# foxcroftjn/polars-strsim

Measured on AMD Instinct MI355X. Metric: M string-pairs/s, levenshtein, 100 M rows (+ achieved HBM GB/s in roofline), higher is better.
Workload: dtype u8/u32 bit-parallel, f64 epilogue

## Files before the change

polars-strsim_amd/csrc/strsim_lane_core.h:

```cpp
#pragma once
#include <stdint.h>
#include <type_traits>

#if defined(__HIPCC__)
#define STRSIM_HD __host__ __device__ __forceinline__
#else
#define STRSIM_HD inline
#endif

namespace strsim {

enum Measure : int { LEVENSHTEIN = 0, JARO = 1, JARO_WINKLER = 2, JACCARD = 3, SORENSEN_DICE = 4 };


#ifndef STRSIM_COLS_PER_TEST
#define STRSIM_COLS_PER_TEST 2
#endif
constexpr int COLS_PER_TEST = STRSIM_COLS_PER_TEST;

STRSIM_HD uint32_t lane_byte(const uint32_t (&w)[8], int j) { return (w[j >> 2] >> ((j & 3) * 8)) & 0xFFu; }

STRSIM_HD uint32_t low_ones(uint32_t k) { return k >= 32u ? 0xFFFFFFFFu : ((1u << k) - 1u); }

template <int G, int NG, typename F>
// ... 101 lines not shown
            const uint32_t t1 = perm_b32(w[2 + h], w[0 + h], 0x07030602u);
            const uint32_t t2 = perm_b32(w[6 + h], w[4 + h], 0x05010400u);
            const uint32_t t3 = perm_b32(w[6 + h], w[4 + h], 0x07030602u);
            r[4 * h + 0] = perm_b32(t2, t0, 0x05040100u);
            r[4 * h + 1] = perm_b32(t2, t0, 0x07060302u);
            r[4 * h + 2] = perm_b32(t3, t1, 0x05040100u);
            r[4 * h + 3] = perm_b32(t3, t1, 0x07060302u);
        }
    }
#pragma unroll
    for (int e = 0; e < 8; e += 2) {
        const uint32_t a = r[e], b = r[e + 1];
        r[e] = bitop3<0xCA>(0x55555555u, a, twice(b));
        r[e + 1] = bitop3<0xCA>(0x55555555u, a >> 1, b);
    }
#pragma unroll
    for (int q = 0; q < 4; ++q) {
        const int e = (q & 1) | ((q & 2) << 1);
        const uint32_t a = r[e], b = r[e + 2];
        r[e] = bitop3<0xCA>(0x33333333u, a, b << 2);
        r[e + 2] = bitop3<0xCA>(0x33333333u, a >> 2, b);
    }
#pragma unroll
    for (int e = 0; e < 4; ++e) {
        const uint32_t a = r[e], b = r[e + 4];
        if (e < NP) P[e < NP ? e : 0] = bitop3<0xCA>(0x0F0F0F0Fu, a, b << 4);
        if (e + 4 < NP) P[e + 4 < NP ? e + 4 : 0] = bitop3<0xCA>(0x0F0F0F0Fu, a >> 4, b);
    }
}

template <int NP>
STRSIM_HD uint32_t eq_mask(const uint32_t (&P)[NP], uint32_t valid, uint32_t w, int byte)
{
    uint32_t acc = valid;
#pragma unroll
    for (int k = 0; k < NP; ++k) acc = bitop3<0x90>(acc, P[k], bit_fill(w, 8 * byte + k));
    return acc;
}

STRSIM_HD int planes_needed(uint32_t vary) { return (vary & 0x40u) ? 7 : ((vary & 0x20u) ? 6 : 5); }

STRSIM_HD uint32_t window_vary(const uint32_t (&wa)[8], const uint32_t (&wb)[8], uint32_t &any)
{
    uint32_t o = bitop3<0xFE>(wa[0], wa[1], wa[2]), n = bitop3<0x80>(wa[0], wa[1], wa[2]);
    o = bitop3<0xFE>(o, wa[3], wa[4]); n = bitop3<0x80>(n, wa[3], wa[4]);
    o = bitop3<0xFE>(o, wa[5], wa[6]); n = bitop3<0x80>(n, wa[5], wa[6]);
    o = bitop3<0xFE>(o, wa[7], wb[0]); n = bitop3<0x80>(n, wa[7], wb[0]);
    o = bitop3<0xFE>(o, wb[1], wb[2]); n = bitop3<0x80>(n, wb[1], wb[2]);
    o = bitop3<0xFE>(o, wb[3], wb[4]); n = bitop3<0x80>(n, wb[3], wb[4]);
    o = bitop3<0xFE>(o, wb[5], wb[6]); n = bitop3<0x80>(n, wb[5], wb[6]);
    o |= wb[7]; n &= wb[7];
    uint32_t o8 = o | (o >> 16); o8 |= o8 >> 8;
    uint32_t n8 = n & (n >> 16); n8 &= n8 >> 8;
    any = o8 & 0xFFu;
    return (o8 ^ n8) & 0xFFu;
}

template <int NP>
STRSIM_HD uint32_t lev_myers32_snap(const uint32_t (&wt)[8], uint32_t lt, uint32_t tmin, uint32_t tmax, const uint32_t (&P)[NP],
                                    uint32_t lp)
{
    uint32_t Pv = 0xFFFFFFFFu, Mv = 0u;
#pragma unroll
    for (int g = 0; g < 32 / COLS_PER_TEST; ++g) {
        if ((uint32_t)(COLS_PER_TEST * g) >= tmax) break;
        auto column = [&](int j) {
            const uint32_t Eq = eq_mask<NP>(P, 0xFFFFFFFFu, wt[j >> 2], j & 3);
            const uint32_t D0 = bitop3<0xBE>((Eq & Pv) + Pv, Pv, Eq) | Mv;
            const uint32_t nHP = bitop3<0x0E>(Mv, D0, Pv);
            const uint32_t nX = twice(nHP);
            const uint32_t HN2 = twice(D0 & Pv);
            Pv = bitop3<0xF2>(HN2, D0, nX);
            Mv = bitop3<0x50>(D0, D0, nX);
        };
        if ((uint32_t)(COLS_PER_TEST * (g + 1)) >= tmin) {
#pragma unroll
            for (int jj = 0; jj < COLS_PER_TEST; ++jj)
                if ((uint32_t)(COLS_PER_TEST * g + jj) < lt) column(COLS_PER_TEST * g + jj);
        } else {
#pragma unroll
            for (int jj = 0; jj < COLS_PER_TEST; ++jj) column(COLS_PER_TEST * g + jj);
        }
    }
    const uint32_t rows = low_ones(lp);
    return lt + popc32(Pv & rows) - popc32(Mv & rows);
}

STRSIM_HD uint32_t common_prefix4(uint32_t a0, uint32_t la, uint32_t b0, uint32_t lb)
{
    const uint32_t x = a0 ^ b0;
    uint32_t p = 4u;
    if (x & 0x000000FFu) p = 0u;
    else if (x & 0x0000FF00u) p = 1u;
    else if (x & 0x00FF0000u) p = 2u;
    else if (x & 0xFF000000u) p = 3u;
    if (p > la) p = la;
    if (p > lb) p = lb;
    return p;
}

STRSIM_HD double epilogue_levenshtein(uint64_t dist, uint64_t la, uint64_t lb)
{
    const uint64_t den = la > lb ? la : lb;
    return 1.0 - ((double)dist / (double)den);
}

STRSIM_HD double epilogue_jaro(uint64_t m, uint64_t t, uint64_t la, uint64_t lb)
{
    if (m == 0) return 0.0;
    const double dm = (double)m;
    return (dm / (double)la + dm / (double)lb + (double)(m - t / 2) / dm) / 3.0;
}

STRSIM_HD double epilogue_jaro_winkler(double jaro, uint32_t prefix)
{
    if (jaro > 0.7) {
        const double pl = (double)prefix;
        return jaro + (pl * 0.1 * (1.0 - jaro));
    }
    return jaro;
}

STRSIM_HD double epilogue_jaccard(uint64_t isect, uint64_t la, uint64_t lb)
{
    return (double)isect / (double)(la + lb - isect);
}

STRSIM_HD double epilogue_sorensen_dice(uint64_t isect, uint64_t la, uint64_t lb)
{
    return 2.0 * (double)isect / (double)(la + lb);
}

template <int NP, bool DO_LEV, bool DO_JARO, bool DO_ISECT, bool KEEP_EQ = false>
STRSIM_HD void lane_cores32(const uint32_t (&wa)[8], uint32_t la, uint32_t tmin, uint32_t tmax, uint32_t lb,
                            const uint32_t (&P)[NP], uint32_t &dist, uint32_t &m_out, uint32_t &t_out, uint32_t &isect)
{
    const uint32_t lbmask = low_ones(lb);
    uint32_t Pv = 0xFFFFFFFFu, Mv = 0u;
    const uint32_t mx = la > lb ? la : lb;
    const uint32_t half = mx >> 1;
    const uint32_t bound = (half ? half : 1u) - 1u;
    uint32_t win = low_ones(bound + 1u);
    uint32_t fb = 0u, fa = 0u;
    const uint32_t valid = DO_JARO ? lbmask : 0xFFFFFFFFu;
    uint32_t used = 0u;
    uint32_t E[(DO_JARO && KEEP_EQ) ? 32 : 1];
#pragma unroll
    for (int g = 0; g < 32 / COLS_PER_TEST; ++g) {
        if ((uint32_t)(COLS_PER_TEST * g) >= tmax) break;
        auto column = [&](int i, bool live) {
            const uint32_t Eq = eq_mask<NP>(P, valid, wa[i >> 2], i & 3);
            if (DO_JARO && KEEP_EQ) E[(DO_JARO && KEEP_EQ) ? i : 0] = Eq;
            if (!live) return;
            if (DO_LEV) {
                const uint32_t D0 = bitop3<0xBE>((Eq & Pv) + Pv, Pv, Eq) | Mv;
                const uint32_t nHP = bitop3<0x0E>(Mv, D0, Pv);
                const uint32_t nX = twice(nHP);
                const uint32_t HN2 = twice(D0 & Pv);
                Pv = bitop3<0xF2>(HN2, D0, nX);
                Mv = bitop3<0x50>(D0, D0, nX);
            }
            if (DO_JARO) {
                const uint32_t cand = bitop3<0x40>(Eq, win, fb);
                fb = bitop3<0xF8>(fb, cand, 0u - cand);
                fa |= cand ? (1u << i) : 0u;
                win = win + win + ((uint32_t)i < bound ? 1u : 0u);
// ... 58 lines not shown
```

polars-strsim_amd/csrc/strsim_lane_stage.h:

```cpp
#pragma once

#ifndef STRSIM_STAGE_ROWS
#define STRSIM_STAGE_ROWS 512
#endif
#ifndef STRSIM_STAGE_CAP
#define STRSIM_STAGE_CAP 10240
#endif
#ifndef STRSIM_STAGE_CAP_LONG
#define STRSIM_STAGE_CAP_LONG 15104
#endif
#ifndef STRSIM_STAGE_CAP_LUT
#define STRSIM_STAGE_CAP_LUT 8960
#endif
#ifndef STRSIM_STAGE_WAVES_PER_EU
#define STRSIM_STAGE_WAVES_PER_EU 5
#endif
#ifndef STRSIM_STAGE_BUCKET_SHIFT
#define STRSIM_STAGE_BUCKET_SHIFT 1
#endif

#ifndef STRSIM_STAGE_LUT
#define STRSIM_STAGE_LUT 0x26
#endif
#ifndef STRSIM_JARO_KEEP_EQ_FILLS
#define STRSIM_JARO_KEEP_EQ_FILLS 1
#endif
#ifndef STRSIM_STAGE_LONG_TEXT_MAX
#define STRSIM_STAGE_LONG_TEXT_MAX 32
#endif
#ifndef STRSIM_STAGE_RANGE_MAX
#define STRSIM_STAGE_RANGE_MAX 64
#endif
#ifndef STRSIM_STAGE_RANGE_DIV
#define STRSIM_STAGE_RANGE_DIV 4
#endif
#ifndef STRSIM_STAGE_RANGE_MIN_BLOCKS
#define STRSIM_STAGE_RANGE_MIN_BLOCKS 2
#endif

#if defined(STRSIM_LAB) && defined(STRSIM_STAGE_STAMPS)
__device__ unsigned long long g_stage_stamps[16384][16];
#define STAGE_STAMP(cat) do { __builtin_amdgcn_sched_barrier(0); const unsigned long long t_ = __builtin_amdgcn_s_memtime(); \
                              __builtin_amdgcn_sched_barrier(0); st_acc[cat] += t_ - st_last; st_last = t_; } while (0)
#else
#define STAGE_STAMP(cat) do { } while (0)
#endif

#ifndef STRSIM_STAGE_THREADS
#define STRSIM_STAGE_THREADS 256
#endif
constexpr int STAGE_BLOCK = STRSIM_STAGE_THREADS;
constexpr int STAGE_WAVES = STAGE_BLOCK / 64;
constexpr int STAGE_ROWS = STRSIM_STAGE_ROWS;
constexpr int STAGE_RPT = STAGE_ROWS / STAGE_BLOCK;
constexpr int STAGE_NR = STAGE_ROWS / 64;
constexpr int STAGE_RPW = STAGE_NR / STAGE_WAVES;
template <int MEASURE> constexpr bool stage_uses_lut() { return ((STRSIM_STAGE_LUT >> MEASURE) & 1) != 0; }

template <bool TABLES, bool LONG = false> struct StageGeom {
    static_assert(!(TABLES && LONG), "the long-row geometry has no match-mask tables");
    static constexpr int CAP = LONG ? STRSIM_STAGE_CAP_LONG : (TABLES ? STRSIM_STAGE_CAP_LUT : STRSIM_STAGE_CAP);
    static constexpr int COL = CAP + 96;
    static constexpr int DMA_ITERS = (CAP + 48 + 16 * STAGE_BLOCK - 1) / (16 * STAGE_BLOCK);
    static_assert(CAP % 16 == 0 && 2 * COL + 64 + 16 <= 65536, "staging area: whole wave-instructions, 16-bit LDS offsets");
};
constexpr int STAGE_BSH = STRSIM_STAGE_BUCKET_SHIFT;
constexpr int STAGE_NBK = (32 >> STAGE_BSH) + 1;
static_assert(STAGE_RPT >= 1 && STAGE_RPT <= 4 && STAGE_RPW >= 1, "STAGE_ROWS is 256, 512 or 1024");
static_assert(STAGE_NBK <= 32, "the bucket scan runs on 32 lanes");

#define STRSIM_LDS_ADDR(p) ((uint32_t)(uintptr_t)((__attribute__((address_space(3))) void *)(p)))

__device__ __forceinline__ void lds_dma_b128(const void *gbase, uint32_t goff, uint32_t lds_dst)
{
    uint32_t keep;
    asm volatile("s_mov_b32 %0, m0\n\ts_mov_b32 m0, %3\n\ts_nop 0\n\tglobal_load_lds_dwordx4 %1, %2\n\ts_mov_b32 m0, %0"
                 : "=&s"(keep)
                 : "v"(goff), "s"(gbase), "s"(lds_dst)
                 : "memory");
}
__device__ __forceinline__ void lds_dma_b32(const void *gbase, uint32_t goff, uint32_t lds_dst)
{
    uint32_t keep;
    asm volatile("s_mov_b32 %0, m0\n\ts_mov_b32 m0, %3\n\ts_nop 0\n\tglobal_load_lds_dword %1, %2\n\ts_mov_b32 m0, %0"
                 : "=&s"(keep)
                 : "v"(goff), "s"(gbase), "s"(lds_dst)
                 : "memory");
}

__device__ __forceinline__ uint32_t load_invariant(const uint32_t *p)
{
    return *reinterpret_cast<const __attribute__((address_space(4))) uint32_t *>(reinterpret_cast<uintptr_t>(p));
}

constexpr uint32_t STAGE_DEAD = 1u << 31;

#if defined(STRSIM_LAB) && defined(STRSIM_STAGE_STRIP)
__device__ const uint16_t *g_strip_ptr;
__global__ __launch_bounds__(256) void k_strip_oracle(const uint32_t *__restrict__ offA, const uint8_t *__restrict__ valA, const uint32_t *__restrict__ offB,
                                                      const uint8_t *__restrict__ valB, uint64_t n, uint16_t *__restrict__ out)
{
    const uint64_t r = (uint64_t)blockIdx.x * 256u + threadIdx.x;
    if (r >= n) return;
    const uint32_t a0 = offA[r], la = offA[r + 1] - a0, b0 = offB[r], lb = offB[r + 1] - b0;
    const uint32_t m = la < lb ? la : lb, cap = (uint32_t)STRSIM_STAGE_STRIP;
    uint32_t p = 0, s = 0;
    while (p < m && p < cap && valA[a0 + p] == valB[b0 + p]) ++p;
    while (s < m - p && s < cap && valA[a0 + la - 1u - s] == valB[b0 + lb - 1u - s]) ++s;
    if (p + s > 63u) s = 63u - p;
    out[r] = (uint16_t)(p | (s << 8));
}
#define STRSIM_STRIP_ON 1
#else
#define STRSIM_STRIP_ON 0
#endif

__device__ __forceinline__ void stage_window(const uint8_t *base, uint32_t at, uint32_t (&w)[8], uint32_t lds_bytes = 0u, uint32_t who = 0u)
{
    typedef uint32_t u32x4_a4 __attribute__((ext_vector_type(4), aligned(4)));
    (void)lds_bytes; (void)who;
    if (who == 1u) STRSIM_CHECK_RANGE(K_STAGE, 40, ~0ull, (at & ~3u) + 36u, 0, lds_bytes);
    if (who == 2u) STRSIM_CHECK_RANGE(K_LIT, 40, ~0ull, (at & ~3u) + 36u, 0, lds_bytes);
    const uint8_t *q = base + (at & ~3u);
    const u32x4_a4 lo = *reinterpret_cast<const u32x4_a4 *>(q);
    const u32x4_a4 hi = *reinterpret_cast<const u32x4_a4 *>(q + 16);
    const uint32_t top = *reinterpret_cast<const uint32_t *>(q + 32);
    const uint32_t sh = at & 3u;
    w[0] = __builtin_amdgcn_alignbyte(lo.y, lo.x, sh); w[1] = __builtin_amdgcn_alignbyte(lo.z, lo.y, sh);
    w[2] = __builtin_amdgcn_alignbyte(lo.w, lo.z, sh); w[3] = __builtin_amdgcn_alignbyte(hi.x, lo.w, sh);
    w[4] = __builtin_amdgcn_alignbyte(hi.y, hi.x, sh); w[5] = __builtin_amdgcn_alignbyte(hi.z, hi.y, sh);
    w[6] = __builtin_amdgcn_alignbyte(hi.w, hi.z, sh); w[7] = __builtin_amdgcn_alignbyte(top, hi.w, sh);
}

__device__ __forceinline__ uint32_t scan32_inclusive(uint32_t x)
{
    x += (uint32_t)__builtin_amdgcn_update_dpp(0, (int)x, 0x111, 0xF, 0xF, true);
    x += (uint32_t)__builtin_amdgcn_update_dpp(0, (int)x, 0x112, 0xF, 0xF, true);
    x += (uint32_t)__builtin_amdgcn_update_dpp(0, (int)x, 0x114, 0xF, 0xF, true);
    x += (uint32_t)__builtin_amdgcn_update_dpp(0, (int)x, 0x118, 0xF, 0xF, true);
    x += (uint32_t)__builtin_amdgcn_update_dpp(0, (int)x, 0x142, 0xA, 0xF, true);
    return x;
}

template <int NP, bool USE_LUT>
__device__ __forceinline__ uint32_t stage_lev_code(const EqLut &lut, const uint32_t (&wa)[8], uint32_t la, const uint32_t (&wb)[8],
                                                   uint32_t lb, uint32_t tmin, uint32_t tmax, uint32_t stripped = 0u)
{
    uint32_t P[NP];
    build_planes<NP>(wb, P);
    EqLut t = lut;
    if (USE_LUT) lut_build<NP>(t, P, 0xFFFFFFFFu);
    const bool live = la != 0u && lb != 0u;
    const uint32_t la1 = live ? la : 1u, lb1 = live ? lb : 1u;
    const uint32_t dist = USE_LUT ? lev_myers32_lut<NP>(t, wa, la1, tmin, tmax, P, lb1) : lev_myers32_snap<NP>(wa, la1, tmin, tmax, P, lb1);
    uint32_t code = dist * (uint32_t)QTAB_N + (la1 > lb1 ? la1 : lb1);
    if (!live) code = (la == 0u && lb == 0u) ? 1u : (uint32_t)QTAB_N + 1u;
#if STRSIM_STRIP_ON
    const uint32_t longer = la > lb ? la : lb;
    code = (live ? dist : longer) * (uint32_t)QTAB_N + (longer + stripped);
#endif
    return code;
}

template <int NP, bool USE_LUT>
__device__ __forceinline__ unsigned long long stage_all_ints(const EqLut &lut, const uint32_t (&wa)[8], uint32_t la,
                                                             const uint32_t (&wb)[8], uint32_t lb, uint32_t tmin, uint32_t tmax)
{
    uint32_t P[NP];
    build_planes<NP>(wb, P);
    const bool live = la != 0u && lb != 0u;
    const uint32_t la1 = live ? la : 1u, lb1 = live ? lb : 1u;
    uint32_t dist, m, t, isect;
    if (USE_LUT) {
        EqLut tb = lut;
        lut_build<NP>(tb, P, 0xFFFFFFFFu);
        lane_cores32_lut<NP, true, true, true>(tb, wa, la1, tmin, tmax, lb1, P, dist, m, t, isect);
    } else {
        lane_cores32<NP, true, true, true>(wa, la1, tmin, tmax, lb1, P, dist, m, t, isect);
    }
    const uint32_t pre = common_prefix4(wa[0], la1, wb[0], lb1);
    const uint32_t lo = dist | (m << 6) | (t << 12) | (isect << 18) | (pre << 24) | (la << 27);
    return (unsigned long long)lo | ((unsigned long long)(la >> 5) << 32) | ((unsigned long long)lb << 33);
}

__device__ __forceinline__ void stage_all_epilogues(unsigned long long pk, double qa, double qb, double qc, double qd, double (&r)[5])
{
    const uint32_t lo = (uint32_t)pk, hi = (uint32_t)(pk >> 32);
    const uint32_t m = (lo >> 6) & 63u, isect = (lo >> 18) & 63u, pre = (lo >> 24) & 7u;
    const uint32_t la = ((lo >> 27) & 31u) | ((hi & 1u) << 5), lb = (hi >> 1) & 63u;
    if (la == 0u || lb == 0u) {
        const double v = (la == 0u && lb == 0u) ? 1.0 : 0.0;
#pragma unroll
        for (int q = 0; q < 5; ++q) r[q] = v;
        return;
    }
    r[LEVENSHTEIN] = 1.0 - qd;
    const double j = m == 0u ? 0.0 : div3_exact(qa + qb + qc);
    r[JARO] = j;
    r[JARO_WINKLER] = epilogue_jaro_winkler(j, pre);
    r[JACCARD] = epilogue_jaccard(isect, la, lb);
    r[SORENSEN_DICE] = epilogue_sorensen_dice(isect, la, lb);
}

template <int MEASURE, int NP, bool USE_LUT>
__device__ __forceinline__ uint32_t stage_ints(const EqLut &lut, const uint32_t (&wa)[8], uint32_t la, const uint32_t (&wb)[8],
                                               uint32_t lb, uint32_t tmin, uint32_t tmax)
{
    uint32_t P[NP];
    build_planes<NP>(wb, P);
    const bool live = la != 0u && lb != 0u;
    const uint32_t la1 = live ? la : 1u, lb1 = live ? lb : 1u;
    uint32_t dist, m, t, isect;
    EqLut tb = lut;
    if (USE_LUT) lut_build<NP>(tb, P, 0xFFFFFFFFu);
    if (MEASURE == JARO || MEASURE == JARO_WINKLER) {
        if (USE_LUT) lane_cores32_lut<NP, false, true, false>(tb, wa, la1, tmin, tmax, lb1, P, dist, m, t, isect);
        else lane_cores32<NP, false, true, false, STRSIM_JARO_KEEP_EQ_FILLS != 0>(wa, la1, tmin, tmax, lb1, P, dist, m, t, isect);
        const uint32_t pre = MEASURE == JARO_WINKLER ? common_prefix4(wa[0], la1, wb[0], lb1) : 0u;
        return m | (t << 6) | (la << 12) | (lb << 18) | (pre << 24);
    }
    if (USE_LUT) lane_cores32_lut<NP, false, false, true>(tb, wa, la1, tmin, tmax, lb1, P, dist, m, t, isect);
    else lane_cores32<NP, false, false, true>(wa, la1, tmin, tmax, lb1, P, dist, m, t, isect);
    return isect | (la << 6) | (lb << 12);
}

template <int MEASURE>
__device__ __forceinline__ double stage_epilogue(uint32_t pk, double qa, double qb, double qc)
{
    if (MEASURE == JARO || MEASURE == JARO_WINKLER) {
        const uint32_t m = pk & 63u, la = (pk >> 12) & 63u, lb = (pk >> 18) & 63u, pre = (pk >> 24) & 7u;
        if (la == 0u || lb == 0u) return (la == 0u && lb == 0u) ? 1.0 : 0.0;
        const double j = m == 0u ? 0.0 : div3_exact(qa + qb + qc);
        return MEASURE == JARO_WINKLER ? epilogue_jaro_winkler(j, pre) : j;
    }
    const uint32_t isect = pk & 63u, la = (pk >> 6) & 63u, lb = (pk >> 12) & 63u;
    if (la == 0u || lb == 0u) return (la == 0u && lb == 0u) ? 1.0 : 0.0;
    return MEASURE == JACCARD ? epilogue_jaccard(isect, la, lb) : epilogue_sorensen_dice(isect, la, lb);
}

template <int MEASURE, bool LUT>
__device__ __forceinline__ void stage_compute(const EqLut &lut, const uint32_t (&wt)[8], const uint32_t (&wp)[8], uint32_t meta,
                                              uint32_t last, uint16_t *s_code, uint32_t *s_word, double *s_val)
{
    bool fast = (meta & STAGE_DEAD) == 0u;
#if STRSIM_STRIP_ON
    const uint32_t lt = meta & 0x3Fu, lp = (meta >> 8) & 0x3Fu, idx = (meta >> 16) & 0x1FFu, stripped = (meta >> 25) & 0x3Fu;
#else
    const uint32_t lt = meta & 0x3Fu, lp = (meta >> 8) & 0x3Fu, idx = (meta >> 16) & 0x7FFu, stripped = 0u;
#endif
    uint32_t any;
    const uint32_t vary = window_vary(wt, wp, any);
    if (any & 0x80u) fast = false;
    if (__ballot(fast) == 0ull) return;
    const uint32_t la = fast ? lt : 0u, lb = fast ? lp : 0u;
    static_assert((1 << STAGE_BSH) % COLS_PER_TEST == 0, "a bucket's upper bound is a whole number of column groups");
    const uint32_t ltl = (uint32_t)__builtin_amdgcn_readlane((int)lt, (int)last);
    const uint32_t tmax = (((ltl ? ltl : 1u) - 1u) | ((1u << STAGE_BSH) - 1u)) + 1u;
    const bool wide = __ballot(fast && (vary & 0x60u)) != 0ull;
    const uint32_t lt0 = uniform(lt);
    const uint32_t tmin = (((lt0 ? lt0 : 1u) - 1u) & ~((1u << STAGE_BSH) - 1u)) + 1u;
    if (MEASURE == LEVENSHTEIN) {
        uint32_t code;
        if (wide) code = stage_lev_code<7, LUT>(lut, wt, la, wp, lb, tmin, tmax, stripped);
        else code = stage_lev_code<5, LUT>(lut, wt, la, wp, lb, tmin, tmax, stripped);
        if (fast) STRSIM_CHECK_INDEX(K_STAGE, 42, ~0ull, idx, STAGE_ROWS);
        if (fast) s_code[idx] = (uint16_t)code;
    } else if (MEASURE == ALL_MEASURES) {
        unsigned long long pk;
        if (wide) pk = stage_all_ints<7, LUT>(lut, wt, la, wp, lb, tmin, tmax);
        else pk = stage_all_ints<5, LUT>(lut, wt, la, wp, lb, tmin, tmax);
        if (fast) STRSIM_CHECK_INDEX(K_STAGE, 43, ~0ull, idx, STAGE_ROWS);
        if (fast) reinterpret_cast<unsigned long long *>(s_val)[idx] = pk;
    } else {
        uint32_t pk;
        if (wide) pk = stage_ints<MEASURE, 7, LUT>(lut, wt, la, wp, lb, tmin, tmax);
        else pk = stage_ints<MEASURE, 5, LUT>(lut, wt, la, wp, lb, tmin, tmax);
        if (fast) STRSIM_CHECK_INDEX(K_STAGE, 44, ~0ull, idx, STAGE_ROWS);
        if (fast) s_word[idx] = pk;
    }
}

template <int MEASURE, bool LUT, bool LONG = false>
__device__ __forceinline__ void
lane_stage_body(const uint32_t *__restrict__ offA, const uint8_t *__restrict__ valA, uint64_t rowsA,
             const uint32_t *__restrict__ offB, const uint8_t *__restrict__ valB, uint64_t rowsB, OutPtrs outs,
             uint64_t n, unsigned long long *__restrict__ slowmask, DevStatus *__restrict__ status,
             const double *__restrict__ qtab, uint32_t *__restrict__ sched, DevStatus *__restrict__ publish, uint32_t ticket)
{
    constexpr bool LEV = MEASURE == LEVENSHTEIN;
    constexpr bool ALL = MEASURE == ALL_MEASURES;
    constexpr int B = STAGE_ROWS, RPT = STAGE_RPT, NBK = STAGE_NBK;
    constexpr int STAGE_CAP = StageGeom<LUT, LONG>::CAP, STAGE_COL = StageGeom<LUT, LONG>::COL;
    constexpr int STAGE_DMA_ITERS = StageGeom<LUT, LONG>::DMA_ITERS;
    constexpr uint32_t COLB = STAGE_COL, LIT = 2u * STAGE_COL;
    static_assert(!LUT || (B <= 128 * STAGE_WAVES && LUT_WAVE_BYTES == 3072), "descriptor slices: 128 rows behind each wave's tables");
    __shared__ __attribute__((aligned(4096))) uint8_t s_lut[LUT ? 4096 * STAGE_WAVES : 16];
    __shared__ uint2 s_desc_own[LUT ? 1 : B];
    __shared__ __attribute__((aligned(4096))) uint8_t s_bytes[2 * STAGE_COL + 64 + 16];
    auto desc_at = [&](uint32_t p) -> uint2 * {
        if (LUT) return reinterpret_cast<uint2 *>(s_lut + ((p >> 7) << 12) + LUT_WAVE_BYTES + ((p & 127u) << 3));
        return s_desc_own + p;
    };
    __shared__ __attribute__((aligned(16))) uint32_t s_off[2][B + 4];
    __shared__ uint32_t s_cnt[32];
    __shared__ uint32_t s_left;
    __shared__ uint32_t s_sched[2];
    __shared__ uint16_t s_code[LEV ? B : 1];
    __shared__ uint32_t s_word[(!LEV && !ALL) ? B : 1];
    __shared__ double s_val[ALL ? B : 1];

    const uint32_t tid = threadIdx.x, lane = lane_id(), wv = tid >> 6;
    if (blockIdx.x == 0u && tid < (uint32_t)(sizeof(DevStatus) / sizeof(uint32_t))) reinterpret_cast<uint32_t *>(status)[tid] = 0u;
    if (tid < 32u) s_cnt[tid] = 0u;
    if (tid == 0u) s_left = 0u;
#pragma unroll
    for (int q = 0; q < RPT; ++q) {
        const uint32_t i = (uint32_t)q * STAGE_BLOCK + tid;
        if (LEV) s_code[i] = 0xFFFFu;
        else if (ALL) reinterpret_cast<unsigned long long *>(&s_val[i])[0] = ~0ull;
        else s_word[i] = 0xFFFFFFFFu;
    }

    const uint32_t totalA = load_invariant(offA + rowsA), totalB = load_invariant(offB + rowsB);
#if STRSIM_BOUNDS_ON
    const uint32_t firstA = load_invariant(offA), firstB = load_invariant(offB);
#endif
    const bool bcastA = rowsA == 1, bcastB = rowsB == 1;
    const uint32_t litA0 = bcastA ? load_invariant(offA) : 0u, litB0 = bcastB ? load_invariant(offB) : 0u;
    const uint32_t litAlen = bcastA ? totalA - litA0 : 0u, litBlen = bcastB ? totalB - litB0 : 0u;
    if (wv == 0u) {
        auto literal_window = [&](const uint8_t *val, uint32_t at, uint32_t total, uint32_t len, uint32_t *dst) {
            uint32_t w[8];
            load_window32(val, at, total, w);
            const uint32_t rep = (w[0] & 0xFFu) * 0x01010101u;
#pragma unroll
            for (int q = 0; q < 8; ++q) {
                const uint32_t v = len > 4u * q ? (len - 4u * q < 4u ? len - 4u * q : 4u) : 0u;
                const uint32_t keep = v >= 4u ? 0xFFFFFFFFu : ((1u << (8u * v)) - 1u);
                dst[q] = (w[q] & keep) | (rep & ~keep);
            }
        };
        if (bcastA) literal_window(valA, litA0, totalA, litAlen, reinterpret_cast<uint32_t *>(s_bytes + LIT));
        if (bcastB) literal_window(valB, litB0, totalB, litBlen, reinterpret_cast<uint32_t *>(s_bytes + LIT + 32u));
    }
    const uint64_t nchunks = (n + 63u) >> 6;
    const uint32_t nchunks32 = (uint32_t)nchunks;
    auto grab = [&](uint32_t seen, uint32_t &lo, uint32_t &sz) {
        const uint32_t left = nchunks32 > seen ? nchunks32 - seen : 0u;
        uint32_t want = (uint32_t)STRSIM_STAGE_RANGE_MAX;
        if (left < (uint32_t)(STRSIM_STAGE_RANGE_MAX * STRSIM_STAGE_RANGE_DIV) * gridDim.x) want = left / ((uint32_t)STRSIM_STAGE_RANGE_DIV * gridDim.x);
        sz = want < (uint32_t)(STRSIM_STAGE_RANGE_MIN_BLOCKS * (B / 64)) ? (uint32_t)(STRSIM_STAGE_RANGE_MIN_BLOCKS * (B / 64)) : want;
        lo = __hip_atomic_fetch_add(&sched[0], sz, __ATOMIC_RELAXED, __HIP_MEMORY_SCOPE_AGENT);
    };
    uint32_t grab_lo = 0u, grab_sz = 0u;
    if (tid == 0u) {
        grab(0u, grab_lo, grab_sz);
        s_sched[0] = grab_lo;
        s_sched[1] = grab_sz;
    }
    lds_barrier();
    uint64_t row_end;
    uint64_t row0;
    {
        const uint64_t lo = uniform(s_sched[0]), hi = lo + uniform(s_sched[1]);
        row0 = lo * 64u < n ? lo * 64u : n;
        row_end = hi * 64u < n ? hi * 64u : n;
    }
    lds_barrier();
    if (tid == 0u) grab(grab_lo, grab_lo, grab_sz);
    bool grab_pending = true;

    EqLut lut;
    lut.lane4 = lane * 4u;
    lut.krep = ((STRSIM_LDS_ADDR(&s_lut[0]) >> 8) + 16u * wv) * 0x01010101u;
    const uint32_t ldsOffA = STRSIM_LDS_ADDR(&s_off[0][0]), ldsOffB = STRSIM_LDS_ADDR(&s_off[1][0]);
    const uint32_t ldsBytes = STRSIM_LDS_ADDR(&s_bytes[0]);
    const uint32_t wvu = uniform(wv);
    const uint32_t tid4 = tid * 4u, tid16 = tid * 16u;
    auto dma_offsets = [&](uint64_t row) {
        const uint32_t cnt = (uint32_t)(row_end - row < (uint64_t)B ? row_end - row : (uint64_t)B);
        const uint32_t *const pa = offA + row, *const pb = offB + row;
#pragma unroll
        for (int it = 0; it < RPT; ++it) {
            if (tid + (uint32_t)it * STAGE_BLOCK <= cnt) {
                if (!bcastA) STRSIM_CHECK_INDEX(K_STAGE, 1, row, row + (uint64_t)it * STAGE_BLOCK + tid, rowsA + 1u);
                if (!bcastB) STRSIM_CHECK_INDEX(K_STAGE, 2, row, row + (uint64_t)it * STAGE_BLOCK + tid, rowsB + 1u);
                STRSIM_CHECK_INDEX(K_STAGE, 3, row, (uint32_t)it * STAGE_BLOCK + tid, B + 4);
                if (!bcastA) lds_dma_b32(pa + it * STAGE_BLOCK, tid4, ldsOffA + 4u * ((uint32_t)it * STAGE_BLOCK + wvu * 64u));
                if (!bcastB) lds_dma_b32(pb + it * STAGE_BLOCK, tid4, ldsOffB + 4u * ((uint32_t)it * STAGE_BLOCK + wvu * 64u));
            }
        }
        if (tid == 0u && cnt == (uint32_t)B) {
            if (!bcastA) STRSIM_CHECK_INDEX(K_STAGE, 4, row, row + (uint64_t)B, rowsA + 1u);
            if (!bcastB) STRSIM_CHECK_INDEX(K_STAGE, 5, row, row + (uint64_t)B, rowsB + 1u);
            if (!bcastA) lds_dma_b32(pa + B, tid4, ldsOffA + 4u * (uint32_t)B);
            if (!bcastB) lds_dma_b32(pb + B, tid4, ldsOffB + 4u * (uint32_t)B);
// ... 91 lines not shown
        }
    };

#if defined(STRSIM_LAB) && defined(STRSIM_STAGE_STAMPS)
    unsigned long long st_acc[10] = {0, 0, 0, 0, 0, 0, 0, 0, 0, 0};
    const unsigned long long st_t0 = __builtin_amdgcn_s_memtime(), st_r0 = __builtin_amdgcn_s_memrealtime();
    unsigned long long st_last = st_t0;
#endif
    while (row0 < row_end) {
        if (grab_pending) {
            if (tid == 0u) {
                s_sched[0] = grab_lo;
                s_sched[1] = grab_sz;
            }
            grab_pending = false;
        }
        if (prev_rows) store_block(prev_row0, prev_rows);
        STAGE_STAMP(1);
        const uint32_t avail = (uint32_t)(row_end - row0 < (uint64_t)B ? row_end - row0 : (uint64_t)B);
        const uint32_t baseA = bcastA ? litA0 : uniform(s_off[0][0]), baseB = bcastB ? litB0 : uniform(s_off[1][0]);
        const uint32_t misA = (uint32_t)(reinterpret_cast<uintptr_t>(valA + baseA) & 15u);
        const uint32_t misB = (uint32_t)(reinterpret_cast<uintptr_t>(valB + baseB) & 15u);
        uint32_t rows;
        {
            const uint32_t e = (lane + 1u) * 64u < avail ? (lane + 1u) * 64u : avail;
            const bool exists = lane * 64u < avail && lane < (uint32_t)(B / 64);
            const uint32_t endA = bcastA ? baseA : s_off[0][exists ? e : 0u], endB = bcastB ? baseB : s_off[1][exists ? e : 0u];
            const bool fits = exists && endA - baseA + misA <= (uint32_t)STAGE_CAP && endB - baseB + misB <= (uint32_t)STAGE_CAP;
            const unsigned long long okm = __ballot(fits);
            uint32_t k = (uint32_t)__builtin_ctzll(~okm);
            if (k == 0u) k = 1u;
            rows = uniform(k * 64u < avail ? k * 64u : avail);
        }
        const uint32_t endA = bcastA ? baseA : uniform(s_off[0][rows]), endB = bcastB ? baseB : uniform(s_off[1][rows]);
        const uint32_t spanA = endA - baseA + misA, spanB = endB - baseB + misB;
        const uint32_t stagedA = bcastA ? 0u : (((spanA < (uint32_t)STAGE_CAP ? spanA : (uint32_t)STAGE_CAP) + 15u) & ~15u);
        const uint32_t stagedB = bcastB ? 0u : (((spanB < (uint32_t)STAGE_CAP ? spanB : (uint32_t)STAGE_CAP) + 15u) & ~15u);
        const uint32_t leftA = totalA - baseA + misA, leftB = totalB - baseB + misB;
        const uint32_t chunksA = bcastA ? 0u : ((stagedA + 32u < leftA ? stagedA + 32u : leftA) + 15u) >> 4;
        const uint32_t chunksB = bcastB ? 0u : ((stagedB + 32u < leftB ? stagedB + 32u : leftB) + 15u) >> 4;
        if (tid < 2u) STRSIM_CHECK_RANGE(K_STAGE, 20, row0, (chunksA << 4) + tid * 16u + 16u, 0, COLB);
        else if (tid < 4u) STRSIM_CHECK_RANGE(K_STAGE, 21, row0, COLB + (chunksB << 4) + (tid - 2u) * 16u + 16u, 0, sizeof(s_bytes));
        if (tid < 2u) *reinterpret_cast<uint4 *>(s_bytes + (chunksA << 4) + tid * 16u) = make_uint4(0u, 0u, 0u, 0u);
        else if (tid < 4u) *reinterpret_cast<uint4 *>(s_bytes + COLB + (chunksB << 4) + (tid - 2u) * 16u) = make_uint4(0u, 0u, 0u, 0u);
        {
            const uint8_t *__restrict__ const gA = valA + baseA - misA, *__restrict__ const gB = valB + baseB - misB;
#pragma unroll
            for (int it = 0; it < STAGE_DMA_ITERS; ++it) {
                if (tid + (uint32_t)it * STAGE_BLOCK < chunksA) {
                    STRSIM_CHECK_COLUMN(K_STAGE, 22, row0, gA + 16 * it * STAGE_BLOCK + tid16, 16, valA, firstA, totalA);
                    STRSIM_CHECK_RANGE(K_STAGE, 23, row0, 16u * ((uint32_t)it * STAGE_BLOCK + tid) + 16u, 0, COLB);
                    lds_dma_b128(gA + 16 * it * STAGE_BLOCK, tid16, ldsBytes + 16u * ((uint32_t)it * STAGE_BLOCK + wvu * 64u));
                }
                if (tid + (uint32_t)it * STAGE_BLOCK < chunksB) {
                    STRSIM_CHECK_COLUMN(K_STAGE, 24, row0, gB + 16 * it * STAGE_BLOCK + tid16, 16, valB, firstB, totalB);
                    STRSIM_CHECK_RANGE(K_STAGE, 25, row0, COLB + 16u * ((uint32_t)it * STAGE_BLOCK + tid) + 16u, 0, sizeof(s_bytes));
                    lds_dma_b128(gB + 16 * it * STAGE_BLOCK, tid16, ldsBytes + COLB + 16u * ((uint32_t)it * STAGE_BLOCK + wvu * 64u));
                }
            }
        }
        STAGE_STAMP(0);
        uint32_t skey[RPT], srank[RPT], sd0[RPT], sd1[RPT];
        {
#pragma unroll
            for (int q = 0; q < RPT; ++q) {
                const uint32_t i = (uint32_t)RPT * tid + (uint32_t)q;
                STRSIM_CHECK_INDEX(K_STAGE, 30, row0, i + 1u, B + 4);
                const bool have = i < rows;
                const uint32_t a0 = bcastA ? 0u : s_off[0][i] - baseA, b0 = bcastB ? 0u : s_off[1][i] - baseB;
                const uint32_t la8 = bcastA ? litAlen : s_off[0][i + 1u] - s_off[0][i];
                const uint32_t lb8 = bcastB ? litBlen : s_off[1][i + 1u] - s_off[1][i];
                const bool stA = bcastA || misA + a0 + la8 <= stagedA, stB = bcastB || misB + b0 + lb8 <= stagedB;
                bool mine = have && la8 <= 32u && lb8 <= 32u && stA && stB;
                if (LONG && STRSIM_STAGE_LONG_TEXT_MAX < 32 && !bcastA && !bcastB) mine = mine && (la8 < lb8 ? la8 : lb8) <= (uint32_t)STRSIM_STAGE_LONG_TEXT_MAX;
                const uint32_t wa = bcastA ? LIT : misA + a0, wb = bcastB ? LIT + 32u : COLB + misB + b0;
                const bool swap = !bcastA && !bcastB && la8 > lb8;
#if STRSIM_STRIP_ON
                uint32_t sp = 0u, ss = 0u;
                if (LEV && !bcastA && !bcastB && have) {
                    const uint32_t ps = g_strip_ptr[row0 + i];
                    sp = ps & 0xFFu; ss = ps >> 8;
                }
                const uint32_t lt = (swap ? lb8 : la8) - sp - ss, lp = (swap ? la8 : lb8) - sp - ss;
                const uint32_t key = mine ? (((lt ? lt : 1u) - 1u) >> STAGE_BSH) : (uint32_t)(NBK - 1);
                skey[q] = key;
                srank[q] = atomicAdd(&s_cnt[key], 1u);
                sd0[q] = mine ? (swap ? ((wb + sp) | ((wa + sp) << 16)) : ((wa + sp) | ((wb + sp) << 16))) : 0u;
                sd1[q] = mine ? (lt | (lp << 8) | (i << 16) | ((sp + ss) << 25)) : STAGE_DEAD;
#else
                const uint32_t lt = swap ? lb8 : la8, lp = swap ? la8 : lb8;
                const uint32_t key = mine ? (((lt ? lt : 1u) - 1u) >> STAGE_BSH) : (uint32_t)(NBK - 1);
                skey[q] = key;
                srank[q] = atomicAdd(&s_cnt[key], 1u);
                sd0[q] = mine ? (swap ? (wb | (wa << 16)) : (wa | (wb << 16))) : 0u;
                sd1[q] = mine ? (lt | (lp << 8) | (i << 16)) : STAGE_DEAD;
#endif
            }
        }
        STAGE_STAMP(2);
        lds_barrier();
        STAGE_STAMP(3);
        uint32_t nmine;
        {
            const uint32_t c = s_cnt[lane & 31u];
            const uint32_t exc = scan32_inclusive(c) - c;
#pragma unroll
            for (int q = 0; q < RPT; ++q) {
                const uint32_t base = __shfl(exc, skey[q], 32);
                const uint32_t p = base + srank[q];
                STRSIM_CHECK_INDEX(K_STAGE, 31, row0, p, B);
                *desc_at(p) = make_uint2(sd0[q], sd1[q]);
            }
            nmine = uniform(__shfl(exc, NBK - 1, 32));
        }
        STAGE_STAMP(4);
        asm volatile("s_waitcnt vmcnt(0)" ::: "memory");
        if (!bcastA && leftA < (chunksA << 4) && tid == ((chunksA - 1u) & (uint32_t)(STAGE_BLOCK - 1)))
            for (uint32_t b = leftA; b < (chunksA << 4); ++b) { STRSIM_CHECK_INDEX(K_STAGE, 32, row0, b, COLB); s_bytes[b] = 0; }
        if (!bcastB && leftB < (chunksB << 4) && tid == ((chunksB - 1u) & (uint32_t)(STAGE_BLOCK - 1)))
            for (uint32_t b = leftB; b < (chunksB << 4); ++b) { STRSIM_CHECK_INDEX(K_STAGE, 33, row0, COLB + b, sizeof(s_bytes)); s_bytes[COLB + b] = 0; }
        lds_barrier();
        STAGE_STAMP(5);
        if (tid < 32u) s_cnt[tid] = 0u;
        uint64_t next_row0 = row0 + rows;
        if (next_row0 >= row_end) {
            const uint64_t lo = uniform(s_sched[0]), hi = lo + uniform(s_sched[1]);
            next_row0 = lo * 64u < n ? lo * 64u : n;
            row_end = hi * 64u < n ? hi * 64u : n;
            if (tid == 0u) grab((uint32_t)lo, grab_lo, grab_sz);
            grab_pending = true;
        }
        if (next_row0 < row_end) dma_offsets(next_row0);
        STAGE_STAMP(6);
        __builtin_amdgcn_s_setprio(0);
        {
            const uint32_t nrounds = (nmine + 63u) >> 6;
#pragma unroll 1
            for (int k = 0; k < STAGE_RPW; ++k) {
                const uint32_t t = (uint32_t)(k >> 1) * (2u * STAGE_WAVES) + ((k & 1) ? (uint32_t)(2 * STAGE_WAVES - 1) - wv : wv);
                if (t >= nrounds) continue;
                const uint32_t hi = nmine - 64u * t;
                const uint32_t first = hi >= 64u ? hi - 64u : 0u;
                const uint32_t in_round = hi - first;
                __builtin_amdgcn_s_setprio(1);
                STRSIM_CHECK_INDEX(K_STAGE, 41, row0, first + lane, B);
                const uint2 d = *desc_at(first + lane);
                uint32_t wt[8], wp[8];
                stage_window(s_bytes, d.x & 0xFFFFu, wt, (uint32_t)sizeof(s_bytes), STRSIM_BOUNDS_ON ? 1u : 0u);
                stage_window(s_bytes, d.x >> 16, wp, (uint32_t)sizeof(s_bytes), STRSIM_BOUNDS_ON ? 1u : 0u);
    #if defined(STRSIM_LAB) && defined(STRSIM_STAGE_STAMPS)
                asm volatile("s_waitcnt lgkmcnt(0)" ::: "memory");
    #endif
                STAGE_STAMP(7);
                __builtin_amdgcn_s_setprio(0);
                stage_compute<MEASURE, LUT>(lut, wt, wp, lane < in_round ? d.y : STAGE_DEAD, in_round - 1u, s_code, s_word, s_val);
                STAGE_STAMP(8);
            }
        }
        __builtin_amdgcn_s_setprio(1);
        asm volatile("s_waitcnt vmcnt(0)" ::: "memory");
        lds_barrier();
        STAGE_STAMP(9);
        prev_row0 = row0;
        prev_rows = rows;
        row0 = next_row0;
    }
    if (prev_rows) store_block(prev_row0, prev_rows);
    if (publish) lds_barrier();
    if (tid == 0u) {
        if (publish && s_left) __hip_atomic_fetch_add(&sched[2], s_left, __ATOMIC_RELAXED, __HIP_MEMORY_SCOPE_AGENT);
        const uint32_t done = __hip_atomic_fetch_add(&sched[1], 1u, __ATOMIC_ACQ_REL, __HIP_MEMORY_SCOPE_AGENT);
        if (done == gridDim.x - 1u) {
            if (publish) {
                const uint32_t total = __hip_atomic_load(&sched[2], __ATOMIC_RELAXED, __HIP_MEMORY_SCOPE_AGENT);
                __hip_atomic_store(&publish->lane_left, total, __ATOMIC_RELEASE, __HIP_MEMORY_SCOPE_SYSTEM);
                if (ticket) __hip_atomic_store(&publish->ticket, ticket, __ATOMIC_RELEASE, __HIP_MEMORY_SCOPE_SYSTEM);
            }
            __hip_atomic_store(&sched[0], 0u, __ATOMIC_RELAXED, __HIP_MEMORY_SCOPE_AGENT);
            __hip_atomic_store(&sched[1], 0u, __ATOMIC_RELAXED, __HIP_MEMORY_SCOPE_AGENT);
            __hip_atomic_store(&sched[2], 0u, __ATOMIC_RELAXED, __HIP_MEMORY_SCOPE_AGENT);
        }
    }
#if defined(STRSIM_LAB) && defined(STRSIM_STAGE_STAMPS)
    if (lane == 0u) {
        const uint32_t w = (blockIdx.x * STAGE_WAVES + wv) & 16383u;
        for (int q = 0; q < 10; ++q) g_stage_stamps[w][q] = st_acc[q];
        g_stage_stamps[w][10] = __builtin_amdgcn_s_memtime() - st_t0;
        const unsigned long long st_r1 = __builtin_amdgcn_s_memrealtime();
        g_stage_stamps[w][11] = st_r1 - st_r0;
        g_stage_stamps[w][12] = st_r0;
        g_stage_stamps[w][13] = st_r1;
        g_stage_stamps[w][14] = (unsigned long long)__builtin_amdgcn_s_getreg((4 << 0) | (0 << 6) | (31 << 11));
        g_stage_stamps[w][15] = (unsigned long long)__builtin_amdgcn_s_getreg((20 << 0) | (0 << 6) | (31 << 11));
    }
#endif
}

#ifndef STRSIM_STAGE_PLAIN_WAVES
#define STRSIM_STAGE_PLAIN_WAVES 5
#endif
#ifndef STRSIM_STAGE_ALL_WAVES_PER_EU
#define STRSIM_STAGE_ALL_WAVES_PER_EU 3
#endif
template <int MEASURE, bool TABLES, bool LONG = false> constexpr int stage_waves_per_eu()
{
    constexpr int lim = MEASURE == ALL_MEASURES ? STRSIM_STAGE_ALL_WAVES_PER_EU : ((TABLES || LONG) ? 4 : STRSIM_STAGE_PLAIN_WAVES);
    return STRSIM_STAGE_WAVES_PER_EU < lim ? STRSIM_STAGE_WAVES_PER_EU : lim;
}

template <int MEASURE, bool TABLES, bool LONG = false>
__global__ __launch_bounds__(STAGE_BLOCK) __attribute__((amdgpu_waves_per_eu(stage_waves_per_eu<MEASURE, TABLES, LONG>()))) void
k_lane_stage(const uint32_t *__restrict__ offA, const uint8_t *__restrict__ valA, uint64_t rowsA,
             const uint32_t *__restrict__ offB, const uint8_t *__restrict__ valB, uint64_t rowsB, OutPtrs outs, uint64_t n,
             unsigned long long *__restrict__ slowmask, DevStatus *__restrict__ status, const double *__restrict__ qtab,
             uint32_t *__restrict__ sched, DevStatus *__restrict__ publish, uint32_t ticket)
{
    lane_stage_body<MEASURE, TABLES, LONG>(offA, valA, rowsA, offB, valB, rowsB, outs, n, slowmask, status, qtab, sched, publish, ticket);
}

__global__ __launch_bounds__(STAGE_BLOCK) __attribute__((amdgpu_waves_per_eu(stage_waves_per_eu<ALL_MEASURES, stage_uses_lut<ALL_MEASURES>()>()))) void
k_lane_stage_all(const uint32_t *__restrict__ offA, const uint8_t *__restrict__ valA, uint64_t rowsA,
                 const uint32_t *__restrict__ offB, const uint8_t *__restrict__ valB, uint64_t rowsB, OutPtrs outs, uint64_t n,
                 unsigned long long *__restrict__ slowmask, DevStatus *__restrict__ status, const double *__restrict__ qtab,
                 uint32_t *__restrict__ sched, DevStatus *__restrict__ publish, uint32_t ticket)
{
    lane_stage_body<ALL_MEASURES, stage_uses_lut<ALL_MEASURES>()>(offA, valA, rowsA, offB, valB, rowsB, outs, n, slowmask, status, qtab, sched, publish, ticket);
}
```

Baseline: 70150.

## Sort Levenshtein rows by exact text length and mask columns per-lane suffix

For the Levenshtein non-LUT path, rows are now bucketed by exact text length (bucket shift 0, 33 buckets with a 64-lane scan) instead of 2-column buckets. The Myers loop becomes a fully unrolled column walk where, past the round's minimum length, each column's active lanes are computed from the bucket boundaries via readlane and an inverse ballot. Lanes whose text is already exhausted stop updating, so per-lane tail checks are replaced by wave-uniform masks. This is meant to tighten the tmin/tmax column range per wave. The cost is a wider count scan, an extra readlane per pair of columns, and loss of the COLS_PER_TEST grouping.

```diff
diff --git a/polars-strsim_amd/csrc/strsim_lane_core.h b/polars-strsim_amd/csrc/strsim_lane_core.h
--- a/polars-strsim_amd/csrc/strsim_lane_core.h
+++ b/polars-strsim_amd/csrc/strsim_lane_core.h
@@ -207,6 +207,40 @@
             for (int jj = 0; jj < COLS_PER_TEST; ++jj) column(COLS_PER_TEST * g + jj);
         }
     }
+    const uint32_t rows = low_ones(lp);
+    return lt + popc32(Pv & rows) - popc32(Mv & rows);
+}
+
+struct TailPerPair {
+    STRSIM_HD bool live(int j, uint32_t lt, uint32_t) { return (uint32_t)j < lt; }
+};
+
+STRSIM_HD unsigned long long suffix_live_mask(uint32_t pair, int j, uint32_t first)
+{
+    const int below = (int)((j & 1) ? pair >> 16 : pair & 0xFFFFu) - (int)first;
+    const int c = below > 0 ? below : 0;
+    return below >= 64 ? 0ull : ~0ull << (uint32_t)c;
+}
+
+template <int NP, typename TAIL>
+STRSIM_HD uint32_t lev_myers32_ordered(const uint32_t (&wt)[8], uint32_t lt, uint32_t tmin, uint32_t tmax, const uint32_t (&P)[NP],
+                                       uint32_t lp, TAIL tail)
+{
+    uint32_t Pv = 0xFFFFFFFFu, Mv = 0u;
+    unrolled_until<0, 32>([&](auto jc) {
+        constexpr int j = decltype(jc)::value;
+        if ((uint32_t)j >= tmax) return false;
+        if (tail.live(j, lt, tmin)) {
+            const uint32_t Eq = eq_mask<NP>(P, 0xFFFFFFFFu, wt[j >> 2], j & 3);
+            const uint32_t D0 = bitop3<0xBE>((Eq & Pv) + Pv, Pv, Eq) | Mv;
+            const uint32_t nHP = bitop3<0x0E>(Mv, D0, Pv);
+            const uint32_t nX = twice(nHP);
+            const uint32_t HN2 = twice(D0 & Pv);
+            Pv = bitop3<0xF2>(HN2, D0, nX);
+            Mv = bitop3<0x50>(D0, D0, nX);
+        }
+        return true;
+    });
     const uint32_t rows = low_ones(lp);
     return lt + popc32(Pv & rows) - popc32(Mv & rows);
 }
diff --git a/polars-strsim_amd/csrc/strsim_lane_stage.h b/polars-strsim_amd/csrc/strsim_lane_stage.h
--- a/polars-strsim_amd/csrc/strsim_lane_stage.h
+++ b/polars-strsim_amd/csrc/strsim_lane_stage.h
@@ -17,6 +17,9 @@
 #endif
 #ifndef STRSIM_STAGE_BUCKET_SHIFT
 #define STRSIM_STAGE_BUCKET_SHIFT 1
+#endif
+#ifndef STRSIM_STAGE_LEV_EXACT
+#define STRSIM_STAGE_LEV_EXACT 1
 #endif
 
 #ifndef STRSIM_STAGE_LUT
@@ -46,6 +49,11 @@
 #define STAGE_STAMP(cat) do { } while (0)
 #endif
 
+#if defined(STRSIM_LAB) && defined(STRSIM_STAGE_STRIP)
+#define STRSIM_STRIP_ON_EARLY 1
+#else
+#define STRSIM_STRIP_ON_EARLY 0
+#endif
 #ifndef STRSIM_STAGE_THREADS
 #define STRSIM_STAGE_THREADS 256
 #endif
@@ -68,6 +76,10 @@
 constexpr int STAGE_NBK = (32 >> STAGE_BSH) + 1;
 static_assert(STAGE_RPT >= 1 && STAGE_RPT <= 4 && STAGE_RPW >= 1, "STAGE_ROWS is 256, 512 or 1024");
 static_assert(STAGE_NBK <= 32, "the bucket scan runs on 32 lanes");
+template <int MEASURE, bool TABLES, bool LONG> constexpr bool stage_exact_order()
+{
+    return STRSIM_STAGE_LEV_EXACT != 0 && MEASURE == LEVENSHTEIN && !TABLES && !LONG && !(STRSIM_STRIP_ON_EARLY);
+}
 
 #define STRSIM_LDS_ADDR(p) ((uint32_t)(uintptr_t)((__attribute__((address_space(3))) void *)(p)))
 
@@ -142,17 +154,42 @@
     return x;
 }
 
-template <int NP, bool USE_LUT>
+__device__ __forceinline__ uint32_t scan64_inclusive(uint32_t x)
+{
+    x = scan32_inclusive(x);
+    x += (uint32_t)__builtin_amdgcn_update_dpp(0, (int)x, 0x143, 0xC, 0xF, true);
+    return x;
+}
+
+struct StageSuffixTail {
+    uint32_t bounds, first;
+    uint32_t pair;
+    __device__ __forceinline__ bool live(int j, uint32_t, uint32_t tmin)
+    {
+        unsigned long long mask = ~0ull;
+        if ((uint32_t)j >= tmin) {
+            if ((j & 1) == 0 || (uint32_t)j == tmin) pair = (uint32_t)__builtin_amdgcn_readlane((int)bounds, j & ~1);
+            mask = suffix_live_mask(pair, j, first);
+        }
+        return __builtin_amdgcn_inverse_ballot_w64(mask);
+    }
+};
+
+template <int NP, bool USE_LUT, bool EXACT = false>
 __device__ __forceinline__ uint32_t stage_lev_code(const EqLut &lut, const uint32_t (&wa)[8], uint32_t la, const uint32_t (&wb)[8],
-                                                   uint32_t lb, uint32_t tmin, uint32_t tmax, uint32_t stripped = 0u)
-{
+                                                   uint32_t lb, uint32_t tmin, uint32_t tmax, uint32_t stripped = 0u,
+                                                   uint32_t bounds = 0u, uint32_t first = 0u)
+{
+    static_assert(!(EXACT && USE_LUT), "the suffix masks are built into the bit-fill core only");
     uint32_t P[NP];
     build_planes<NP>(wb, P);
     EqLut t = lut;
     if (USE_LUT) lut_build<NP>(t, P, 0xFFFFFFFFu);
     const bool live = la != 0u && lb != 0u;
     const uint32_t la1 = live ? la : 1u, lb1 = live ? lb : 1u;
-    const uint32_t dist = USE_LUT ? lev_myers32_lut<NP>(t, wa, la1, tmin, tmax, P, lb1) : lev_myers32_snap<NP>(wa, la1, tmin, tmax, P, lb1);
+    uint32_t dist;
+    if constexpr (EXACT) dist = lev_myers32_ordered<NP>(wa, la1, tmin, tmax, P, lb1, StageSuffixTail{bounds, first, 0u});
+    else dist = USE_LUT ? lev_myers32_lut<NP>(t, wa, la1, tmin, tmax, P, lb1) : lev_myers32_snap<NP>(wa, la1, tmin, tmax, P, lb1);
     uint32_t code = dist * (uint32_t)QTAB_N + (la1 > lb1 ? la1 : lb1);
     if (!live) code = (la == 0u && lb == 0u) ? 1u : (uint32_t)QTAB_N + 1u;
 #if STRSIM_STRIP_ON
@@ -238,10 +275,13 @@
     return MEASURE == JACCARD ? epilogue_jaccard(isect, la, lb) : epilogue_sorensen_dice(isect, la, lb);
 }
 
-template <int MEASURE, bool LUT>
+template <int MEASURE, bool LUT, bool EXACT = false>
 __device__ __forceinline__ void stage_compute(const EqLut &lut, const uint32_t (&wt)[8], const uint32_t (&wp)[8], uint32_t meta,
-                                              uint32_t last, uint16_t *s_code, uint32_t *s_word, double *s_val)
-{
+                                              uint32_t last, uint16_t *s_code, uint32_t *s_word, double *s_val,
+                                              uint32_t bounds = 0u, uint32_t first = 0u)
+{
+    static_assert(!EXACT || MEASURE == LEVENSHTEIN, "exact length order: Levenshtein only");
+    constexpr int BSH = EXACT ? 0 : STAGE_BSH;
     bool fast = (meta & STAGE_DEAD) == 0u;
 #if STRSIM_STRIP_ON
     const uint32_t lt = meta & 0x3Fu, lp = (meta >> 8) & 0x3Fu, idx = (meta >> 16) & 0x1FFu, stripped = (meta >> 25) & 0x3Fu;
@@ -253,16 +293,16 @@
     if (any & 0x80u) fast = false;
     if (__ballot(fast) == 0ull) return;
     const uint32_t la = fast ? lt : 0u, lb = fast ? lp : 0u;
-    static_assert((1 << STAGE_BSH) % COLS_PER_TEST == 0, "a bucket's upper bound is a whole number of column groups");
+    static_assert((1 << BSH) % (EXACT ? 1 : COLS_PER_TEST) == 0, "a bucket's upper bound is a whole number of column groups");
     const uint32_t ltl = (uint32_t)__builtin_amdgcn_readlane((int)lt, (int)last);
-    const uint32_t tmax = (((ltl ? ltl : 1u) - 1u) | ((1u << STAGE_BSH) - 1u)) + 1u;
+    const uint32_t tmax = (((ltl ? ltl : 1u) - 1u) | ((1u << BSH) - 1u)) + 1u;
     const bool wide = __ballot(fast && (vary & 0x60u)) != 0ull;
     const uint32_t lt0 = uniform(lt);
-    const uint32_t tmin = (((lt0 ? lt0 : 1u) - 1u) & ~((1u << STAGE_BSH) - 1u)) + 1u;
+    const uint32_t tmin = (((lt0 ? lt0 : 1u) - 1u) & ~((1u << BSH) - 1u)) + 1u;
     if (MEASURE == LEVENSHTEIN) {
         uint32_t code;
-        if (wide) code = stage_lev_code<7, LUT>(lut, wt, la, wp, lb, tmin, tmax, stripped);
-        else code = stage_lev_code<5, LUT>(lut, wt, la, wp, lb, tmin, tmax, stripped);
+        if (wide) code = stage_lev_code<7, LUT, EXACT>(lut, wt, la, wp, lb, tmin, tmax, stripped, bounds, first);
+        else code = stage_lev_code<5, LUT, EXACT>(lut, wt, la, wp, lb, tmin, tmax, stripped, bounds, first);
         if (fast) STRSIM_CHECK_INDEX(K_STAGE, 42, ~0ull, idx, STAGE_ROWS);
         if (fast) s_code[idx] = (uint16_t)code;
     } else if (MEASURE == ALL_MEASURES) {
@@ -289,7 +329,9 @@
 {
     constexpr bool LEV = MEASURE == LEVENSHTEIN;
     constexpr bool ALL = MEASURE == ALL_MEASURES;
-    constexpr int B = STAGE_ROWS, RPT = STAGE_RPT, NBK = STAGE_NBK;
+    constexpr bool EXACT = stage_exact_order<MEASURE, LUT, LONG>();
+    constexpr int B = STAGE_ROWS, RPT = STAGE_RPT, BSH = EXACT ? 0 : STAGE_BSH, NBK = (32 >> BSH) + 1;
+    constexpr int NCNT = NBK <= 32 ? 32 : 64;
     constexpr int STAGE_CAP = StageGeom<LUT, LONG>::CAP, STAGE_COL = StageGeom<LUT, LONG>::COL;
     constexpr int STAGE_DMA_ITERS = StageGeom<LUT, LONG>::DMA_ITERS;
     constexpr uint32_t COLB = STAGE_COL, LIT = 2u * STAGE_COL;
@@ -302,7 +344,7 @@
         return s_desc_own + p;
     };
     __shared__ __attribute__((aligned(16))) uint32_t s_off[2][B + 4];
-    __shared__ uint32_t s_cnt[32];
+    __shared__ uint32_t s_cnt[NCNT];
     __shared__ uint32_t s_left;
     __shared__ uint32_t s_sched[2];
     __shared__ uint16_t s_code[LEV ? B : 1];
@@ -311,7 +353,7 @@
 
     const uint32_t tid = threadIdx.x, lane = lane_id(), wv = tid >> 6;
     if (blockIdx.x == 0u && tid < (uint32_t)(sizeof(DevStatus) / sizeof(uint32_t))) reinterpret_cast<uint32_t *>(status)[tid] = 0u;
-    if (tid < 32u) s_cnt[tid] = 0u;
+    if (tid < (uint32_t)NCNT) s_cnt[tid] = 0u;
     if (tid == 0u) s_left = 0u;
 #pragma unroll
     for (int q = 0; q < RPT; ++q) {
@@ -569,14 +611,14 @@
                     sp = ps & 0xFFu; ss = ps >> 8;
                 }
                 const uint32_t lt = (swap ? lb8 : la8) - sp - ss, lp = (swap ? la8 : lb8) - sp - ss;
-                const uint32_t key = mine ? (((lt ? lt : 1u) - 1u) >> STAGE_BSH) : (uint32_t)(NBK - 1);
+                const uint32_t key = mine ? (((lt ? lt : 1u) - 1u) >> BSH) : (uint32_t)(NBK - 1);
                 skey[q] = key;
                 srank[q] = atomicAdd(&s_cnt[key], 1u);
                 sd0[q] = mine ? (swap ? ((wb + sp) | ((wa + sp) << 16)) : ((wa + sp) | ((wb + sp) << 16))) : 0u;
                 sd1[q] = mine ? (lt | (lp << 8) | (i << 16) | ((sp + ss) << 25)) : STAGE_DEAD;
 #else
                 const uint32_t lt = swap ? lb8 : la8, lp = swap ? la8 : lb8;
-                const uint32_t key = mine ? (((lt ? lt : 1u) - 1u) >> STAGE_BSH) : (uint32_t)(NBK - 1);
+                const uint32_t key = mine ? (((lt ? lt : 1u) - 1u) >> BSH) : (uint32_t)(NBK - 1);
                 skey[q] = key;
                 srank[q] = atomicAdd(&s_cnt[key], 1u);
                 sd0[q] = mine ? (swap ? (wb | (wa << 16)) : (wa | (wb << 16))) : 0u;
@@ -588,17 +630,20 @@
         lds_barrier();
         STAGE_STAMP(3);
         uint32_t nmine;
+        uint32_t bounds = 0u;
         {
-            const uint32_t c = s_cnt[lane & 31u];
-            const uint32_t exc = scan32_inclusive(c) - c;
+            const uint32_t c = s_cnt[lane & (uint32_t)(NCNT - 1)];
+            const uint32_t inc = NCNT == 64 ? scan64_inclusive(c) : scan32_inclusive(c);
+            const uint32_t exc = inc - c;
 #pragma unroll
             for (int q = 0; q < RPT; ++q) {
-                const uint32_t base = __shfl(exc, skey[q], 32);
+                const uint32_t base = __shfl(exc, skey[q], NCNT);
                 const uint32_t p = base + srank[q];
                 STRSIM_CHECK_INDEX(K_STAGE, 31, row0, p, B);
                 *desc_at(p) = make_uint2(sd0[q], sd1[q]);
             }
-            nmine = uniform(__shfl(exc, NBK - 1, 32));
+            nmine = uniform(__shfl(exc, NBK - 1, NCNT));
+            if (EXACT) bounds = exc | (inc << 16);
         }
         STAGE_STAMP(4);
         asm volatile("s_waitcnt vmcnt(0)" ::: "memory");
@@ -608,7 +653,7 @@
             for (uint32_t b = leftB; b < (chunksB << 4); ++b) { STRSIM_CHECK_INDEX(K_STAGE, 33, row0, COLB + b, sizeof(s_bytes)); s_bytes[COLB + b] = 0; }
         lds_barrier();
         STAGE_STAMP(5);
-        if (tid < 32u) s_cnt[tid] = 0u;
+        if (tid < (uint32_t)NCNT) s_cnt[tid] = 0u;
         uint64_t next_row0 = row0 + rows;
         if (next_row0 >= row_end) {
             const uint64_t lo = uniform(s_sched[0]), hi = lo + uniform(s_sched[1]);
@@ -640,7 +685,7 @@
     #endif
                 STAGE_STAMP(7);
                 __builtin_amdgcn_s_setprio(0);
-                stage_compute<MEASURE, LUT>(lut, wt, wp, lane < in_round ? d.y : STAGE_DEAD, in_round - 1u, s_code, s_word, s_val);
+                stage_compute<MEASURE, LUT, EXACT>(lut, wt, wp, lane < in_round ? d.y : STAGE_DEAD, in_round - 1u, s_code, s_word, s_val, bounds, uniform(first));
                 STAGE_STAMP(8);
             }
         }
```

After: 70820 (median of 6 runs). Within noise of the previous version (+1.0%).
